# andreaskoepf/faster-rcnn.torch

Measured on AMD Instinct MI355X. Metric: images/sec (vgg_small 800x450 fwd+bwd), higher is better.
Workload: dtype f32 (conv / Linear(13824,1024) operands as 2 x fp16 split planes: 22 significand bits, 3 MFMA partial products; fp32 accumulate)

## Files before the change

### faster-rcnn.torch_amd/csrc/convx.hip

```cpp
#include <cstdlib>

#include "kernels.h"
#include "amax.h"
#include <type_traits>
#ifdef CX_TRACE
#include <cstdio>
#include <vector>
#endif

namespace frcnn {

typedef float f32x16 __attribute__((ext_vector_type(16)));
typedef __bf16 bf16x8 __attribute__((ext_vector_type(8)));
typedef __bf16 bf16x2 __attribute__((ext_vector_type(2)));
typedef float f32x2 __attribute__((ext_vector_type(2)));
typedef _Float16 f16x8 __attribute__((ext_vector_type(8)));
typedef _Float16 f16x2 __attribute__((ext_vector_type(2)));

#define CX_BM 128
#define CX_CH 16
#define CX_OCC 3
#define CX_PP 204
constexpr int cx_pp(int k) { return k == 3 ? CX_PP : k == 5 ? 240 : 308; }
#define CX_NA 2
// ... 946 lines not shown
  int grid = a.tilesX * a.tilesY * a.mTiles * a.splitK;
  if (grid > AMAX_MAX_BLOCKS) a.amax_out = nullptr;
#ifdef CX_TRACE
  static unsigned long long* tbuf = nullptr;
  const char* tfile = getenv("FRCNN_X3_TRACE");
  if (tfile && !tbuf) FR_HIP(hipMalloc(&tbuf, 8192 * 512));
  a.trace = tfile && grid <= 8192 ? tbuf : nullptr;
  if (a.trace) FR_HIP(hipMemsetAsync(tbuf, 0, (size_t)grid * 512, s));
#endif
  double bytes = 4.0 * ((double)a.Cin * a.H * a.W + (double)a.M * a.Ho * a.Wo);
  const size_t lds = std::max<size_t>((size_t)cx_ring(NP) * (2 * NP * 64 * WM * 16) + (size_t)CX_NB * (2 * NP * cx_pp(KS) * 16), a.wide ? 4 * 64 * 32 * 4 : 0);
  FR_LAUNCH(KC_CONV_X3, flops, bytes, s, (conv_x3_kernel<KS, WM, SLOPE, SCALE, EPI, NP>), dim3(grid), dim3(256), lds, a);
  FR_LAUNCH_CHECK();
#ifdef CX_TRACE
  if (a.trace) {
    FR_HIP(hipStreamSynchronize(s));
    std::vector<unsigned long long> hst((size_t)grid * 64);
    FR_HIP(hipMemcpy(hst.data(), tbuf, hst.size() * 8, hipMemcpyDeviceToHost));
    if (FILE* f = fopen(tfile, "w")) {
      fprintf(f, "# grid %d M %d Cin %d Ho %d Wo %d TH %d TW %d splitK %d wide %d WM %d EPI %d\n", grid, a.M, a.Cin, a.Ho, a.Wo, a.TH, a.TW, a.splitK, a.wide, WM, EPI);
      for (int b = 0; b < grid; ++b) {
        for (int j = 0; j < 64; ++j) fprintf(f, "%llu ", hst[(size_t)b * 64 + j]);
        fprintf(f, "\n");
      }
      fclose(f);
    }
  }
#endif
  return FRCNN_OK;
}

int conv_x3(const float* in, int Cin, int H, int W, const float* in_slope, const float* in_scale, const void* wp,
            const float* bias, int M, int k, int pad, float* out, int out_mode, double algo_flops, hipStream_t s, int ws_slot,
            const X3PostAct* post, const float* amax_in, const float* amax_w, float* amax_out) {
  FR_CHECK((k == 3 || k == 5 || k == 7) && Cin % CX_CH == 0 && M % 64 == 0,
           "conv_x3: %d channels -> %d filters, %dx%d is not a split-bf16 shape", Cin, M, k, k);
  FR_CHECK((double)Cin * H * W * 4.0 < 4294967295.0, "conv_x3: input tensor too large for 32-bit offsets");
  CxArgs a;
  a.in = in; a.in_slope = in_slope; a.in_scale = in_scale; a.wp = wp; a.bias = bias; a.out = out;
  a.amax_in = amax_in; a.amax_w = amax_w; a.amax_out = amax_out;
  const bool f16 = amax_in != nullptr;
  FR_CHECK(!f16 || amax_w, "conv_x3: the two-plane fp16 form needs the magnitudes of both tensors");
  a.Cin = Cin; a.H = H; a.W = W; a.M = M; a.pad = pad;
  a.Ho = H + 2 * pad - k + 1; a.Wo = W + 2 * pad - k + 1;
  FR_CHECK(a.Ho > 0 && a.Wo > 0, "conv_x3: empty output (%dx%d, k=%d, pad=%d)", H, W, k, pad);
  x3_choose_tile(a.Ho, a.Wo, k, &a.TH, &a.TW);
  a.tilesX = cdiv(a.Wo, a.TW); a.tilesY = cdiv(a.Ho, a.TH);
  const int bm = conv_x3_bm(M, a.Ho, a.Wo, k);
  a.mTiles = M / bm;
  a.nChunks = Cin / CX_CH;
  const long blocks = (long)a.tilesX * a.tilesY * a.mTiles;
  const int min_chunks = cdiv(36, k * k);
  const long slots = 256 * (k == 3 ? CX_OCC : 2);
  int splitK = (int)std::min<long>(std::min<long>(std::max<long>(1, slots / blocks), k == 3 ? 16 : 24), std::max(1, a.nChunks / min_chunks));
  a.chunksPerSplit = cdiv(a.nChunks, splitK);
  a.splitK = cdiv(a.nChunks, a.chunksPerSplit);
  a.out_mode = out_mode;
  a.post = post ? *post : X3PostAct{nullptr, nullptr, nullptr, nullptr};
  a.wide = 0;
  FR_CHECK(!post || (k == 3 && out_mode == OUT_STORE && !in_slope && !in_scale && !bias && post->x && post->slope),
           "conv_x3: the fused activation backward belongs to a storing 3x3 input-gradient launch");
  bool slab = false;
  if (a.splitK > 1) {
    float* ws = nullptr;
    FR_TRY(x3_workspace((size_t)a.splitK * M * a.Ho * a.Wo * 4, &ws, ws_slot & 7));
    a.out = ws; a.out_mode = 3; a.bias = nullptr; slab = true;
    a.amax_out = nullptr;
  }
  a.wide = a.Wo % 4 == 0 && a.TW % 4 == 0 && ((uintptr_t)a.out & 15) == 0 &&
           (!post || ((uintptr_t)post->x & 15) == 0);
  if (algo_flops <= 0) algo_flops = 2.0 * M * Cin * k * k * (double)a.Ho * a.Wo;
  int rc;
  const int act = (in_slope ? 2 : 0) | (in_scale ? 1 : 0);
  if (f16 && k != 3) {
    FR_CHECK(act == 0 && bm == 128, "conv_x3: a %dx%d launch takes no fused input activation and 128-filter blocks", k, k);
    rc = k == 5 ? launch_x3<5, 2, false, false, 0, 2>(a, algo_flops, s) : launch_x3<7, 2, false, false, 0, 2>(a, algo_flops, s);
  } else if (f16) {
    if (post && a.splitK == 1)
      rc = bm == 128 ? launch_x3<3, 2, false, false, 1, 2>(a, algo_flops, s) : launch_x3<3, 1, false, false, 1, 2>(a, algo_flops, s);
    else if (bm == 128)
      rc = act == 3 ? launch_x3<3, 2, true, true, 0, 2>(a, algo_flops, s) : act == 2 ? launch_x3<3, 2, true, false, 0, 2>(a, algo_flops, s)
         : act == 1 ? launch_x3<3, 2, false, true, 0, 2>(a, algo_flops, s) : launch_x3<3, 2, false, false, 0, 2>(a, algo_flops, s);
    else
      rc = act == 3 ? launch_x3<3, 1, true, true, 0, 2>(a, algo_flops, s) : act == 2 ? launch_x3<3, 1, true, false, 0, 2>(a, algo_flops, s)
         : act == 1 ? launch_x3<3, 1, false, true, 0, 2>(a, algo_flops, s) : launch_x3<3, 1, false, false, 0, 2>(a, algo_flops, s);
  } else if (post && a.splitK == 1) {
    rc = bm == 128 ? launch_x3<3, 2, false, false, 1>(a, algo_flops, s) : launch_x3<3, 1, false, false, 1>(a, algo_flops, s);
  } else if (k == 3 && bm == 128) {
    rc = act == 3 ? launch_x3<3, 2, true, true>(a, algo_flops, s) : act == 2 ? launch_x3<3, 2, true, false>(a, algo_flops, s)
       : act == 1 ? launch_x3<3, 2, false, true>(a, algo_flops, s) : launch_x3<3, 2, false, false>(a, algo_flops, s);
  } else if (k == 3) {
    rc = act == 3 ? launch_x3<3, 1, true, true>(a, algo_flops, s) : act == 2 ? launch_x3<3, 1, true, false>(a, algo_flops, s)
       : act == 1 ? launch_x3<3, 1, false, true>(a, algo_flops, s) : launch_x3<3, 1, false, false>(a, algo_flops, s);
  } else {
    FR_CHECK(act == 0 && bm == 128, "conv_x3: a %dx%d launch takes no fused input activation and 128-filter blocks", k, k);
    rc = k == 5 ? launch_x3<5, 2, false, false>(a, algo_flops, s) : launch_x3<7, 2, false, false>(a, algo_flops, s);
  }
  FR_TRY(rc);
  if (amax_out && !slab && (long)a.tilesX * a.tilesY * a.mTiles > AMAX_MAX_BLOCKS)
    FR_TRY(tensor_absmax(out, (long)M * a.Ho * a.Wo, amax_out, s));
  if (slab) {
    long total = (long)M * a.Ho * a.Wo;
    int grid;
    const long hw = (long)a.Ho * a.Wo;
    const X3PostAct pa = post ? *post : X3PostAct{nullptr, nullptr, nullptr, nullptr};
    const bool al = ((uintptr_t)out & 15) == 0 && ((uintptr_t)a.out & 15) == 0 && (!post || ((uintptr_t)post->x & 15) == 0);
    const int vec = al && hw % 4 == 0 ? 4 : al && hw % 2 == 0 ? 2 : 1;
    grid = (int)std::min<long>(cdivl(total / vec, 256), 4096);
    if (vec == 4)
      FR_LAUNCH(KC_ELEMWISE, 0, total * 4.0 * (a.splitK + 1), s, x3_splitk_reduce_kernel<4>, dim3(grid), dim3(256), 0,
                (const float*)a.out, a.splitK, M, hw, bias, out, out_mode == OUT_ADD ? 1 : 0, pa, amax_out);
    else if (vec == 2)
      FR_LAUNCH(KC_ELEMWISE, 0, total * 4.0 * (a.splitK + 1), s, x3_splitk_reduce_kernel<2>, dim3(grid), dim3(256), 0,
                (const float*)a.out, a.splitK, M, hw, bias, out, out_mode == OUT_ADD ? 1 : 0, pa, amax_out);
    else
      FR_LAUNCH(KC_ELEMWISE, 0, total * 4.0 * (a.splitK + 1), s, x3_splitk_reduce_kernel<1>, dim3(grid), dim3(256), 0,
                (const float*)a.out, a.splitK, M, hw, bias, out, out_mode == OUT_ADD ? 1 : 0, pa, amax_out);
    FR_LAUNCH_CHECK();
  }
  return FRCNN_OK;
}

}
```

### faster-rcnn.torch_amd/csrc/elem.hip

```cpp
#include <algorithm>

#include <mutex>
#include <unordered_map>

#include "kernels.h"
#include "amax.h"

namespace frcnn {

__device__ __forceinline__ float wave_sum(float v) {
#pragma unroll
  for (int o = 32; o > 0; o >>= 1) v += __shfl_down(v, o, 64);
  return v;
}

__device__ __forceinline__ float block_sum(float v, float* sh) {
  v = wave_sum(v);
  const int lane = threadIdx.x & 63, w = threadIdx.x >> 6;
  if (lane == 0) sh[w] = v;
  __syncthreads();
  float r = 0.f;
  if (threadIdx.x < 64) {
    r = threadIdx.x < (blockDim.x >> 6) ? sh[threadIdx.x] : 0.f;
    r = wave_sum(r);
// ... 285 lines not shown
  *out = e.first;
  return FRCNN_OK;
}

static int act_bwd_chunks(int C, long hw) {
  long want = cdivl(512, C);
  long maxc = cdivl(hw, 4096);
  return (int)std::max<long>(1, std::min<long>(want, maxc));
}

int maxpool_act_backward(const float* gpool, const unsigned char* idx, const float* x, int C, int H,
                         int W, const float* slope, const float* scale, float* gx, float* gbias,
                         float* gslope, hipStream_t s, float* amax) {
  int Ho = (H - 2 + 1) / 2 + 1, Wo = (W - 2 + 1) / 2 + 1;
  int chunks = act_bwd_chunks(C, (long)H * W);
  float* const amax_after = (amax && (long)C * chunks > AMAX_MAX_BLOCKS) ? amax : nullptr;
  if (amax_after) amax = nullptr;
  float *pb = nullptr, *pa = nullptr;
  if (deterministic()) { FR_TRY(det_workspace(s, (size_t)2 * C * chunks, &pb)); pa = pb + (size_t)C * chunks; }
  const bool vec = (W % 4 == 0) && (Wo % 2 == 0) && (((uintptr_t)gpool | (uintptr_t)x | (uintptr_t)gx) % 16 == 0) &&
                   ((uintptr_t)idx % 2 == 0);
  if (vec)
    FR_LAUNCH(KC_ELEMWISE, 0, (double)C * H * W * 9.25, s, (act_backward_kernel<true, true>), dim3(C * chunks),
              dim3(ACT_BWD_THREADS), 0, gpool, idx, x, C, H, W, Ho, Wo, slope, scale, gx, gbias, gslope, chunks, pb, pa, amax);
  else
    FR_LAUNCH(KC_ELEMWISE, 0, (double)C * H * W * 9.25, s, (act_backward_kernel<true, false>), dim3(C * chunks),
              dim3(ACT_BWD_THREADS), 0, gpool, idx, x, C, H, W, Ho, Wo, slope, scale, gx, gbias, gslope, chunks, pb, pa, amax);
  FR_LAUNCH_CHECK();
  if (pb) FR_TRY(fold_partials(gbias ? pb : nullptr, (slope && gslope) ? pa : nullptr, C, chunks, gbias, gslope, s));
  if (amax_after) FR_TRY(tensor_absmax(gx, (long)C * H * W, amax_after, s));
  return FRCNN_OK;
}

int act_backward(const float* gy, const float* x, int C, long hw, const float* slope,
                 const float* scale, float* gx, float* gbias, float* gslope, hipStream_t s, float* amax) {
  int chunks = act_bwd_chunks(C, hw);
  float* const amax_after = (amax && (long)C * chunks > AMAX_MAX_BLOCKS) ? amax : nullptr;
  if (amax_after) amax = nullptr;
  float *pb = nullptr, *pa = nullptr;
  if (deterministic()) { FR_TRY(det_workspace(s, (size_t)2 * C * chunks, &pb)); pa = pb + (size_t)C * chunks; }
  const bool vec = (hw % 4 == 0) && (((uintptr_t)gy | (uintptr_t)x | (uintptr_t)gx) % 16 == 0);
  if (vec)
    FR_LAUNCH(KC_ELEMWISE, 0, (double)C * hw * 12.0, s, (act_backward_kernel<false, true>), dim3(C * chunks),
              dim3(ACT_BWD_THREADS), 0, gy, (const unsigned char*)nullptr, x, C, 1, (int)hw, 1, 1, slope, scale, gx,
              gbias, gslope, chunks, pb, pa, amax);
  else
    FR_LAUNCH(KC_ELEMWISE, 0, (double)C * hw * 12.0, s, (act_backward_kernel<false, false>), dim3(C * chunks),
              dim3(ACT_BWD_THREADS), 0, gy, (const unsigned char*)nullptr, x, C, 1, (int)hw, 1, 1, slope, scale, gx,
              gbias, gslope, chunks, pb, pa, amax);
  FR_LAUNCH_CHECK();
  if (pb) FR_TRY(fold_partials(gbias ? pb : nullptr, (slope && gslope) ? pa : nullptr, C, chunks, gbias, gslope, s));
  if (amax_after) FR_TRY(tensor_absmax(gx, (long)C * hw, amax_after, s));
  return FRCNN_OK;
}

__global__ void channel_sum_kernel(const float* __restrict__ g, long hw, float* gbias, int chunks, float* part_b) {
  __shared__ float sh[16];
  const int c = blockIdx.x / chunks, chunk = blockIdx.x % chunks;
  long per = cdivl(hw, chunks);
  per = (per + 3) & ~3L;
  const long beg = chunk * per, end = beg + per < hw ? beg + per : hw;
  const float* gc = g + (size_t)c * hw;
  float sb = 0.f;
  if (beg < end) {
    if ((reinterpret_cast<uintptr_t>(gc + beg) & 15) == 0) {
      const long n4 = (end - beg) >> 2;
// ... 586 lines not shown
```

### faster-rcnn.torch_amd/csrc/kernels.h

```cpp
#pragma once
#include <algorithm>

#include "common.h"

namespace frcnn {

int conv_cc(int k);
int conv_mpad(int M);
size_t conv_pack_floats(int Kchan, int M, int k);
int conv_pack_weights(const float* w, int O, int C, int k, float* wf, float* wd, hipStream_t s);
struct PackJob { long w_off; long total; float* dst; int O, C, k, mode, Mpad, blk_begin, nblk; };
PackJob conv_pack_job(long w_off, int O, int C, int k, int mode, float* dst);
int conv_pack_assign_blocks(PackJob* jobs, int njobs, int total_blocks);
int conv_pack_weights_multi(const float* weights, const PackJob* jobs_dev, int njobs, int grid, hipStream_t s);

enum { OUT_STORE = 0, OUT_ADD = 1 };
struct IgemmPool { float* out; unsigned char* idx; const float* slope; const float* scale; float* amax = nullptr; };
int conv_igemm(const float* in, int Cin, int H, int W, const float* in_slope, const float* in_scale,
               const float* wp, const float* bias, int M, int k, int pad, float* out, int out_mode,
               double algo_flops, hipStream_t s, int ws_slot = 0,
               const IgemmPool* pool = nullptr, bool* pool_fused = nullptr);

void set_split_bf16(int on);
int get_split_bf16();
bool conv_x3_eligible(int Cin, int M, int k);
size_t conv_x3_pack_bytes(int Kchan, int M, int k);
struct PackXJob {
  long w_off; long total; void* dst; const float* amax; float* amax_w; int O, C, k, mode, bm, blk_begin, nblk;
  const int* oidx = nullptr; const int* cidx = nullptr; int Cs = 0; long bias_off = 0; float* bias_dst = nullptr;
};
PackXJob conv_x3_pack_job(long w_off, int O, int C, int k, int mode, void* dst, int Ho, int Wo);
int conv_x3_pack_assign_blocks(PackXJob* jobs, int njobs);
int conv_x3_pack_multi(const float* weights, const PackXJob* jobs_dev, int njobs, int grid, hipStream_t s);
int conv_x3_pack(const float* w, int O, int C, int k, int mode, void* dst, hipStream_t s, int Ho, int Wo,
                 const float* amax_rec_w = nullptr, float* amax_w = nullptr);
#define AMAX_REC 16400
#define AMAX_MAX_BLOCKS 16384
int tensor_absmax(const float* x, long n, float* rec, hipStream_t s);
struct AmaxJob { long off; long n; float* out; int blk_begin; };
int tensor_absmax_assign_blocks(AmaxJob* jobs, int njobs);
long tensor_absmax_record_floats(long n);
int tensor_absmax_multi(const float* w, const AmaxJob* jobs_dev, int njobs, int grid, hipStream_t s);
void set_x3_f16(int on);
int get_x3_f16();
int conv_x3(const float* in, int Cin, int H, int W, const float* in_slope, const float* in_scale, const void* wp,
            const float* bias, int M, int k, int pad, float* out, int out_mode, double algo_flops, hipStream_t s, int ws_slot = 0,
            const struct X3PostAct* post = nullptr, const float* amax_in = nullptr, const float* amax_w = nullptr,
            float* amax_out = nullptr);
struct X3PostAct {
  const float* x;
  const float* slope;
  const float* scale;
  float* gslope;
};

bool conv_wgradx_eligible(int Cin, int O, int k);
size_t conv_wgradx_workspace_bytes(int Cin, int H, int W, int O, int pad);
struct WgradMap { const int* omap = nullptr; const int* cmap = nullptr; int Cfull = 0; };
int conv_wgradx(const float* in, int Cin, int H, int W, const float* in_slope, const float* in_scale, const float* g, int O,
                int pad, float* gw, void* ws, size_t ws_bytes, hipStream_t s, float* gbias = nullptr,
                const float* amax_in = nullptr, const float* amax_g = nullptr,
                const WgradMap* map = nullptr);
int wgrad_reduce(const float* slab, int nSplit, int taps, int OC, float* gw, hipStream_t s);
int wgrad_reduce_map(const float* slab, int nSplit, int taps, int O, int C, float* gw, const WgradMap& map, hipStream_t s);
bool conv_wgrad_first_pooled_eligible(int Cin, int O, int k, int Wo);
int conv_wgrad_first_pooled(const float* in, int Cin, int H, int W, const float* gpool, const unsigned char* pidx, const float* x,
                            const float* slope, int O, int pad, float* gw, float* gbias, float* gslope, void* ws, size_t ws_bytes,
                            hipStream_t s);

size_t conv_wgrad_workspace_bytes(int Cin, int H, int W, int O, int k, int pad);
int conv_wgrad(const float* in, int Cin, int H, int W, const float* in_slope, const float* in_scale,
               const float* g, int O, int k, int pad, float* gw, void* ws, size_t ws_bytes, hipStream_t s,
               float* gbias = nullptr,
               const float* amax_in = nullptr, const float* amax_g = nullptr,
               const WgradMap* map = nullptr);

bool deterministic();
void set_deterministic(bool on);
int det_workspace(hipStream_t s, size_t floats, float** out);

int fill_zero(void* p, size_t bytes, hipStream_t s);
int scale_inplace(float* x, long n, float sc, hipStream_t s);
int add_inplace(float* y, const float* x, long n, hipStream_t s);
int act_forward(const float* x, int C, long hw, const float* slope, const float* scale, float* y,
                hipStream_t s);
int maxpool_act_forward(const float* x, int C, int H, int W, const float* slope, const float* scale,
                        float* out, unsigned char* idx, hipStream_t s, float* amax = nullptr);
// ... 191 lines not shown
```

### faster-rcnn.torch_amd/csrc/net.cpp

```cpp
#include <array>
#include <vector>
#include <cmath>
#include <cstring>

#include "kernels.h"

namespace frcnn {

static const int HEAD_OUT = 18;
static const int SPARSE_MAX_POS = 512;

struct DevBuf {
  void* p = nullptr;
  size_t bytes = 0;
  bool owned = true;
  void view(void* ptr, size_t n) { p = ptr; bytes = n; owned = false; }
  int ensure(size_t need) {
    if (need <= bytes) return FRCNN_OK;
    if (p && owned) (void)hipFree(p);
    owned = true;
    p = nullptr; bytes = 0;
    FR_HIP(hipMalloc(&p, need + 64));
    bytes = need;
    return FRCNN_OK;
// ... 48 lines not shown
  int in, n;
  bool bn;
  float p_drop;
  long w_off, b_off, bnw_off, bnb_off, a_off;
  DevBuf lin, pre, post, xhat, invstd, mask, g;
  DevBuf gin;
  DevBuf xp, xpT, gp, gpT;
  int x_form = 0;
  DevBuf am;
  const float* am_w_of = nullptr;
  long am_w_gen = -1;
};

}

using namespace frcnn;

static int g_drop_compact = -1;
static int drop_compact_on() {
  if (g_drop_compact < 0) g_drop_compact = getenv("FRCNN_DROP_COMPACT") ? (atoi(getenv("FRCNN_DROP_COMPACT")) != 0) : 1;
  return g_drop_compact;
}
static int pool_stream(int slot, hipStream_t* out) {
  static hipStream_t pool[8] = {};
  if (!pool[slot]) FR_HIP(hipStreamCreateWithFlags(&pool[slot], hipStreamNonBlocking));
  *out = pool[slot];
  return FRCNN_OK;
}

static int g_sparse_heads = -1;
static int sparse_heads_on() {
  if (g_sparse_heads < 0) g_sparse_heads = getenv("FRCNN_SPARSE_HEADS") ? (atoi(getenv("FRCNN_SPARSE_HEADS")) != 0) : 1;
  return g_sparse_heads;
}
static int g_static_weights = 0;
static long g_static_gen = 0;

struct frcnn_model {
  frcnn_model_desc d;
  std::vector<Conv> convs;
  std::vector<Block> blocks;
  std::vector<Head> heads;
  std::vector<ClsLayer> cls;
  long pnet_params = 0, total_params = 0;
  long bbox_w_off = 0, bbox_b_off = 0, clsw_off = 0, clsb_off = 0;
  int H = 0, W = 0;
  int training = 0;
  DevBuf delta_last;
  DevBuf zero_arena;
  size_t delta_bytes = 0, gpool_bytes = 0;
  DevBuf pack_jobs;
  DevBuf x3_jobs;
  DevBuf amax, amax_ws, amax_jobs;
  int n_amax = 0, n_amax_jobs = 0, amax_grid = 0;
  float* rec(int id) const { return (float*)amax.p + (size_t)id * AMAX_REC; }
  std::vector<unsigned char> am_live;
  float* rec_w(int id) { am_live[id] = 1; return rec(id); }
  void weights_live(bool heads_too) {
    for (auto& c : convs) if (c.x_f || c.x_d) am_live[c.am + 2] = 1;
    for (auto& hd : heads) if (heads_too && (hd.c3.x_f || hd.c3.x_d)) am_live[hd.c3.am + 2] = 1;
  }
  bool f16_packed = false;
  long eval_packs_gen = -1;
  const float* eval_packs_w = nullptr;
  int n_x3_all = 0, n_x3_fwd = 0, x3_grid_all = 0, x3_grid_fwd = 0;
  int n_pack_fwd = 0, n_pack_all = 0, n_pack_heads = 0, pack_grid_fwd = 0, pack_grid_all = 0, pack_grid_heads = 0;
// ... 528 lines not shown
  if (!m->upd_join_ev) FR_HIP(hipEventCreateWithFlags(&m->upd_join_ev, hipEventDisableTiming));
  return FRCNN_OK;
}
int frcnn_model_update_stream(frcnn_model* m, void** stream) {
  FR_CHECK(m && stream, "model_update_stream: null argument");
  FR_TRY(ensure_update_stream(m));
  m->update_armed = true;
  *stream = (void*)m->cw;
  return FRCNN_OK;
}
int frcnn_model_update_fork(frcnn_model* m, void* stream) {
  FR_CHECK(m != nullptr, "model_update_fork: null model");
  FR_TRY(ensure_update_stream(m));
  FR_HIP(hipEventRecord(m->upd_ev, S(stream)));
  FR_HIP(hipStreamWaitEvent(m->cw, m->upd_ev, 0));
  return FRCNN_OK;
}
int frcnn_model_update_join(frcnn_model* m, void* stream) {
  FR_CHECK(m != nullptr, "model_update_join: null model");
  FR_TRY(ensure_update_stream(m));
  FR_HIP(hipEventRecord(m->upd_join_ev, m->cw));
  FR_HIP(hipStreamWaitEvent(S(stream), m->upd_join_ev, 0));
  return FRCNN_OK;
}

int frcnn_get_option(const char* name, int* value) {
  FR_CHECK(name != nullptr && value != nullptr, "get_option: null argument");
  if (strcmp(name, "side_stream") == 0) { *value = side_enabled() ? 1 : 0; return FRCNN_OK; }
  if (strcmp(name, "gemm_x_roles") == 0) { *value = get_gemm_x_roles(); return FRCNN_OK; }
  if (strcmp(name, "deterministic") == 0) { *value = deterministic() ? 1 : 0; return FRCNN_OK; }
  if (strcmp(name, "static_weights") == 0) { *value = g_static_weights; return FRCNN_OK; }
  if (strcmp(name, "drop_compact") == 0) { *value = drop_compact_on(); return FRCNN_OK; }
  if (strcmp(name, "sparse_heads") == 0) { *value = sparse_heads_on(); return FRCNN_OK; }
  if (strcmp(name, "winograd") == 0) { *value = 0; return FRCNN_OK; }
  if (strcmp(name, "cnet_wgrad_async") == 0) { *value = g_cnet_wgrad_async; return FRCNN_OK; }
  if (strcmp(name, "split_bf16") == 0) { *value = get_split_bf16(); return FRCNN_OK; }
  if (strcmp(name, "x3_f16") == 0) { *value = get_x3_f16(); return FRCNN_OK; }
  FR_CHECK(false, "get_option: unknown option '%s'", name);
  return FRCNN_OK;
}

int frcnn_set_option(const char* name, int value) {
  FR_CHECK(name != nullptr, "set_option: null name");
  if (strcmp(name, "side_stream") == 0) { g_side_stream = value ? 1 : 0; return FRCNN_OK; }
  if (strcmp(name, "deterministic") == 0) { set_deterministic(value != 0); return FRCNN_OK; }
  if (strcmp(name, "static_weights") == 0) { g_static_weights = value != 0; ++g_static_gen; return FRCNN_OK; }
  if (strcmp(name, "drop_compact") == 0) { g_drop_compact = value != 0; return FRCNN_OK; }
  if (strcmp(name, "sparse_heads") == 0) { g_sparse_heads = value != 0; return FRCNN_OK; }
  if (strcmp(name, "gemm_x_roles") == 0) { set_gemm_x_roles(value); return FRCNN_OK; }
  if (strcmp(name, "split_bf16") == 0) { set_split_bf16(value); return FRCNN_OK; }
  if (strcmp(name, "x3_f16") == 0) { set_x3_f16(value); return FRCNN_OK; }
  if (strcmp(name, "winograd") == 0) return FRCNN_OK;
  if (strcmp(name, "cnet_wgrad_async") == 0) { g_cnet_wgrad_async = value ? 1 : 0; return FRCNN_OK; }
  FR_CHECK(false, "set_option: unknown option '%s'", name);
  return FRCNN_OK;
}

static int ensure_head_streams(frcnn_model* m);
static int ensure_side(frcnn_model* m) {
  if (!m->side) {
    FR_TRY(pool_stream(0, &m->side));
    FR_HIP(hipEventCreateWithFlags(&m->join_ev, hipEventDisableTiming));
    FR_HIP(hipEventCreateWithFlags(&m->loss_ev, hipEventDisableTiming));
    FR_HIP(hipEventCreateWithFlags(&m->chain_ev, hipEventDisableTiming));
    for (auto& h : m->heads) FR_HIP(hipEventCreateWithFlags(&h.done, hipEventDisableTiming));
  }
  return FRCNN_OK;
}

static int ensure_head_streams(frcnn_model* m) {
  static const int head_streams = getenv("FRCNN_HEAD_STREAMS") ? atoi(getenv("FRCNN_HEAD_STREAMS")) : 1;
  size_t hi = 0;
  for (auto& h : m->heads) {
    if (head_streams && hi < 5 && !h.stream) FR_TRY(pool_stream(2 + (int)hi, &h.stream));
    ++hi;
  }
  return FRCNN_OK;
}

static hipStream_t head_stream(frcnn_model* m, size_t i) { return m->heads[i].stream ? m->heads[i].stream : m->side; }
static int head_slot(frcnn_model* m, size_t i) { return m->heads[i].stream ? 2 + (int)(i % 5) : 1; }
// ... 330 lines not shown
    } break;
    case 4: {
      FR_CHECK(index >= 0 && index < (int)m->blocks.size() && m->H > 0 && m->blocks[index].has_drop, "debug_buffer: block %d has no dropout", index);
      const Block& k = m->blocks[index]; b = &k.scale; n = (size_t)m->d.filters[index] * 4;
    } break;
    case 1: {
      FR_CHECK(index >= 0 && index < (int)m->blocks.size() && m->H > 0, "debug_buffer: block %d (after a forward pass)", index);
      const Block& k = m->blocks[index]; b = &k.pidx; n = (size_t)m->d.filters[index] * k.Hp * k.Wp;
    } break;
    case 2: {
      FR_CHECK(index >= 0 && index < (int)m->heads.size() && m->H > 0, "debug_buffer: anchor net %d (after a forward pass)", index);
      const Conv& c = m->heads[index].c3; b = &c.x; n = (size_t)c.Cout * c.Ho * c.Wo * 4;
      if ((m->heads_sparse_fwd || m->heads_deferred) && m->last_w) {
        FR_HIP(hipDeviceSynchronize());
        if (!m->head_x3_fresh) { FR_TRY(refresh_group(m, m->last_w, (int)m->blocks.size(), nullptr)); m->head_x3_fresh = true; }
        FR_TRY(head_forward(m, m->heads[index], m->last_w, nullptr, 0));
        FR_HIP(hipDeviceSynchronize());
      }
    } break;
    case 3: {
      FR_CHECK(index >= 0 && index < (int)m->cls.size() && m->R > 0, "debug_buffer: classification layer %d (after frcnn_cnet_forward)", index);
      const ClsLayer& L = m->cls[index]; b = L.bn ? &L.pre : &L.lin; n = (size_t)m->R * L.n * 4;
    } break;
    case 7: case 11: {
      FR_CHECK(index >= 0 && index < (int)m->convs.size() && m->H > 0, "debug_buffer: backbone convolution %d (after a forward pass)", index);
      const Conv& c = m->convs[index];
      const Block& k = m->blocks[c.block];
      b = kind == 7 ? &c.x : &c.gx; n = (size_t)((k.dc_on && c.step == 0) ? k.nkM : c.Cout) * c.Ho * c.Wo * 4;
    } break;
    case 9: {
      FR_CHECK(index >= 0 && index < (int)m->blocks.size() && m->H > 0, "debug_buffer: block %d (after a forward pass)", index);
      const Block& k = m->blocks[index]; b = &k.pooled; n = (size_t)m->d.filters[index] * k.Hp * k.Wp * 4;
    } break;
    case 5: case 6: case 8: case 10: {
      const int nc = (int)m->convs.size();
      int id = -1;
      FR_CHECK(m->H > 0, "debug_buffer: magnitude records exist after a forward pass");
      if (kind == 6) {
        FR_CHECK(index >= 0 && index < (int)m->blocks.size(), "debug_buffer: block %d out of range", index);
        id = m->blocks[index].am;
      } else if (kind == 10) {
        FR_CHECK(index >= 0 && index < nc + (int)m->heads.size(), "debug_buffer: weight tensor %d out of range", index);
        id = (index < nc ? m->convs[index].am : m->heads[index - nc].c3.am) + 2;
      } else {
        FR_CHECK(index >= 0 && index < nc, "debug_buffer: backbone convolution %d out of range", index);
        id = m->convs[index].am + (kind == 8 ? 1 : 0);
      }
      FR_CHECK(id >= 0 && id < (int)m->am_live.size() && m->am_live[id], "debug_buffer: the last pass kept no magnitude record of kind %d, index %d", kind, index);
      *ptr = m->rec(id); *bytes = (long long)AMAX_REC * 4;
      return FRCNN_OK;
    }
    default: FR_CHECK(false, "debug_buffer: unknown kind %d", kind);
  }
  FR_CHECK(b->p && b->bytes >= n, "debug_buffer: buffer not allocated yet");
  *ptr = b->p; *bytes = (long long)n;
  return FRCNN_OK;
}

int frcnn_pnet_delta(frcnn_model* m, int i, float** ptr) {
  FR_CHECK(m->H > 0, "pnet_delta: call frcnn_pnet_forward first");
  FR_CHECK(i >= 1 && i <= (int)m->heads.size() + 1, "pnet_delta: index %d out of range", i);
  *ptr = i <= (int)m->heads.size() ? m->heads[i - 1].delta.f() : m->delta_last.f();
  return FRCNN_OK;
}

int frcnn_pnet_set_sparse_deltas(frcnn_model* m, int head, const int* positions, int count) {
// ... 416 lines not shown
      for (auto& h : m->heads) any = any || h.sp_count != 0;
      if (any) FR_TRY(heads_forward_dense(m, w, s));
      m->heads_deferred = false;
    }
    FR_TRY(join_side(m, s));
    if (backbone_trained(m)) FR_TRY(fill_zero((char*)m->zero_arena.p + m->delta_bytes, m->gpool_bytes, s));
    FR_TRY(backward_heads(m, w, grad, s, 0));
  }
  const int fb = m->frozen_blocks;
  if (fb < nb) {
    if (!m->train_heads) FR_TRY(fill_zero((char*)m->zero_arena.p + m->delta_bytes, m->gpool_bytes, s));
    Block& last = m->blocks.back();
    FR_TRY(add_inplace(last.gpooled.f(), m->delta_last.f(), (long)m->d.filters[nb - 1] * last.Hp * last.Wp, s));
  }
  if (m->update_armed) {
    if (!m->bwd_ev) FR_HIP(hipEventCreateWithFlags(&m->bwd_ev, hipEventDisableTiming));
    FR_HIP(hipEventRecord(m->bwd_ev, s));
  }
  for (int b = 0; b < fb; ++b) {
    while (m->block_ev.size() < (size_t)nb) {
      hipEvent_t e;
      FR_HIP(hipEventCreateWithFlags(&e, hipEventDisableTiming));
      m->block_ev.push_back(e);
    }
    FR_HIP(hipEventRecord(m->block_ev[b], s));
    FR_TRY(record_block_read(m, b, s));
  }
  const bool use_side = side_enabled();
  if (use_side) FR_TRY(ensure_side(m));
  hipStream_t ws = use_side ? m->side : s;
  size_t n_fork = 0;
  const bool fuse_act = !deterministic() && !(getenv("FRCNN_FUSE_ACT") && atoi(getenv("FRCNN_FUSE_ACT")) == 0);
  bool act_done = false;
  for (int b = nb - 1; b >= fb; --b) {
    Block& blk = m->blocks[b];
    for (int st = blk.nconv - 1; st >= 0; --st) {
      Conv& c = m->convs[blk.first_conv + st];
      const float* scale = (st == 0 && blk.has_drop) ? blk.scale.f() : nullptr;
      const bool fused_here = act_done;
      act_done = false;
      static const bool first_pooled_on = !(getenv("FRCNN_FIRST_POOLED") && atoi(getenv("FRCNN_FIRST_POOLED")) == 0);
      const bool first_pooled = fuse_act && first_pooled_on && b == 0 && st == 0 && blk.nconv == 1 && scale == nullptr &&
                                conv_wgrad_first_pooled_eligible(c.Cin, c.Cout, c.k, c.Wo);
      if (first_pooled) {
        FR_TRY(conv_wgrad_first_pooled(m->img.f(), c.Cin, c.H, c.W, blk.gpooled.f(), (const unsigned char*)blk.pidx.p, c.x.f(),
                                       w + c.a_off, c.Cout, c.pad, grad + c.w_off, grad + c.b_off, grad + c.a_off,
                                       m->wg_ws_first.p, m->wg_ws_first.bytes, s));
        while (m->block_ev.size() < (size_t)nb) {
          hipEvent_t e;
          FR_HIP(hipEventCreateWithFlags(&e, hipEventDisableTiming));
          m->block_ev.push_back(e);
        }
        FR_HIP(hipEventRecord(m->block_ev[b], s));
        FR_TRY(record_block_read(m, b, s));
        break;
      }
      if (fused_here) {
      } else if (st == blk.nconv - 1) {
        FR_TRY(maxpool_act_backward(blk.gpooled.f(), (const unsigned char*)blk.pidx.p, c.x.f(), c.Cout, c.Ho, c.Wo,
                                    w + c.a_off, scale, c.gx.f(), grad + c.b_off, grad + c.a_off, s,
                                    (c.x_d && m->f16_packed) ? m->rec_w(c.am + 1) : nullptr));
      } else {
        FR_TRY(act_backward(c.gx.f(), c.x.f(), c.Cout, (long)c.Ho * c.Wo, w + c.a_off, scale, c.gx.f(),
                            grad + c.b_off, grad + c.a_off, s, (c.x_d && m->f16_packed) ? m->rec_w(c.am + 1) : nullptr));
      }
      const float* in; const float* in_slope = nullptr; const float* in_scale = nullptr;
      if (st > 0) {
        Conv& pc = m->convs[blk.first_conv + st - 1];
        in = pc.x.f(); in_slope = w + pc.a_off;
        in_scale = (st - 1 == 0 && blk.has_drop) ? blk.scale.f() : nullptr;
      } else {
        in = b == 0 ? m->img.f() : m->blocks[b - 1].pooled.f();
      }
      const bool dc = blk.dc_on && st <= 1;
      int wg_cin = c.Cin, wg_o = c.Cout;
      WgradMap wmap;
      if (dc) {
        wmap.Cfull = c.Cin;
        if (st == 1) { wg_cin = blk.nkM; wmap.cmap = blk.dc_idx; in_scale = nullptr; }
        else { wg_o = blk.nkM; wmap.omap = blk.dc_idx; }
      }
      const float* wa_in = nullptr; const float* wa_g = nullptr;
      if (m->f16_packed && c.x_f && c.x_d && (st > 0 || b > 0)) {
        wa_in = st > 0 ? m->rec(m->convs[blk.first_conv + st - 1].am) : m->rec(m->blocks[b - 1].am);
        wa_g = m->rec(c.am + 1);
      }
      const bool on_caller = use_side && b == 0 && st == 0;
      if (use_side && !on_caller) FR_TRY(fork_side(m, s, n_fork++));
      if (on_caller) {
        FR_TRY(conv_wgrad(in, wg_cin, c.H, c.W, in_slope, in_scale, c.gx.f(), wg_o, c.k, c.pad, grad + c.w_off, m->wg_ws_first.p,
                          m->wg_ws_first.bytes, s, fused_here ? grad + c.b_off : nullptr, wa_in, wa_g, dc ? &wmap : nullptr));
        FR_HIP(hipEventRecord(m->join_ev, ws));
        FR_HIP(hipStreamWaitEvent(s, m->join_ev, 0));
      } else {
        FR_TRY(conv_wgrad(in, wg_cin, c.H, c.W, in_slope, in_scale, c.gx.f(), wg_o, c.k, c.pad, grad + c.w_off, m->wg_ws.p, m->wg_ws.bytes, ws,
                          fused_here ? grad + c.b_off : nullptr, wa_in, wa_g, dc ? &wmap : nullptr));
      }
      if (st == 0) {
        while (m->block_ev.size() < (size_t)nb) {
          hipEvent_t e;
          FR_HIP(hipEventCreateWithFlags(&e, hipEventDisableTiming));
          m->block_ev.push_back(e);
        }
        FR_HIP(hipEventRecord(m->block_ev[b], on_caller ? s : ws));
      }
      if (b == fb && st == 0) {
        FR_TRY(record_block_read(m, b, s));
        break;
      }
      float* gin = st > 0 ? m->convs[blk.first_conv + st - 1].gx.f() : m->blocks[b - 1].gpooled.f();
      const int gmode = st > 0 ? OUT_STORE : OUT_ADD;
      const float* ag = nullptr;
      const float* aw = nullptr;
      if (c.x_d && m->f16_packed) { ag = m->rec(c.am + 1); aw = m->amax_ws.f() + c.am; }
      const int dg_k = (dc && st == 0) ? blk.nkK : c.Cout, dg_m = (dc && st == 1) ? blk.nkM : c.Cin;
      const double fl = 2.0 * dg_k * dg_m * c.k * c.k * (double)c.Ho * c.Wo;
      if (c.x_d && st > 0 && fuse_act && c.k == 3) {
        Conv& pc = m->convs[blk.first_conv + st - 1];
        X3PostAct post{pc.x.f(), w + pc.a_off, (st - 1 == 0 && blk.has_drop && !dc) ? blk.scale.f() : nullptr, grad + pc.a_off};
        FR_TRY(conv_x3(c.gx.f(), dg_k, c.Ho, c.Wo, nullptr, nullptr, c.wxd.p, nullptr, dg_m, c.k, c.k - 1 - c.pad, gin, gmode, fl, s, 0, &post, ag, aw,
                       (pc.x_d && m->f16_packed) ? m->rec_w(pc.am + 1) : nullptr));
        act_done = true;
      } else if (c.x_d)
        FR_TRY(conv_x3(c.gx.f(), dg_k, c.Ho, c.Wo, nullptr, nullptr, c.wxd.p, nullptr, dg_m, c.k, c.k - 1 - c.pad, gin, gmode, fl, s, 0, nullptr, ag, aw));
      else
        FR_TRY(conv_igemm(c.gx.f(), c.Cout, c.Ho, c.Wo, nullptr, nullptr, c.wd.f(), nullptr, c.Cin, c.k,
                          c.k - 1 - c.pad, gin, gmode, fl, s));
      if (st == 0) FR_TRY(record_block_read(m, b, s));
    }
  }
  m->block_ev_valid = true;
  if (heads_tail && !m->heads_gin) FR_TRY(join_heads(m, s));
  FR_TRY(cw_join(m, s));
  if (use_side) {
    FR_HIP(hipEventRecord(m->join_ev, ws));
    FR_HIP(hipStreamWaitEvent(s, m->join_ev, 0));
    m->side_busy = false;
  }
  return FRCNN_OK;
}

static bool cnet_fuse() {
  const char* e = getenv("FRCNN_CNET_FUSE");
  return !(e && atoi(e) == 0);
}
static bool gemm_f16_on() {
  static const bool env_on = !(getenv("FRCNN_GEMM_F16") && atoi(getenv("FRCNN_GEMM_F16")) == 0);
  return env_on && get_x3_f16();
}
static int ensure_cnet(frcnn_model* m, int R) {
  for (auto& L : m->cls) {
    size_t n = (size_t)R * L.n * 4;
    FR_TRY(L.lin.ensure(n));
    if (L.bn) { FR_TRY(L.pre.ensure(n)); FR_TRY(L.xhat.ensure(n)); FR_TRY(L.invstd.ensure((size_t)L.n * 4)); }
    FR_TRY(L.post.ensure(n));
// ... 227 lines not shown
```

Before: 510.9.

## Fuse split-K slab reduction with maxpool and activation backward at block boundaries

```diff
diff --git a/faster-rcnn.torch_amd/csrc/convx.hip b/faster-rcnn.torch_amd/csrc/convx.hip
--- a/faster-rcnn.torch_amd/csrc/convx.hip
+++ b/faster-rcnn.torch_amd/csrc/convx.hip
@@ -1002,7 +1002,7 @@
 
 int conv_x3(const float* in, int Cin, int H, int W, const float* in_slope, const float* in_scale, const void* wp,
             const float* bias, int M, int k, int pad, float* out, int out_mode, double algo_flops, hipStream_t s, int ws_slot,
-            const X3PostAct* post, const float* amax_in, const float* amax_w, float* amax_out) {
+            const X3PostAct* post, const float* amax_in, const float* amax_w, float* amax_out, X3PoolBack* pool) {
   FR_CHECK((k == 3 || k == 5 || k == 7) && Cin % CX_CH == 0 && M % 64 == 0,
            "conv_x3: %d channels -> %d filters, %dx%d is not a split-bf16 shape", Cin, M, k, k);
   FR_CHECK((double)Cin * H * W * 4.0 < 4294967295.0, "conv_x3: input tensor too large for 32-bit offsets");
@@ -1030,6 +1030,8 @@
   a.wide = 0;
   FR_CHECK(!post || (k == 3 && out_mode == OUT_STORE && !in_slope && !in_scale && !bias && post->x && post->slope),
            "conv_x3: the fused activation backward belongs to a storing 3x3 input-gradient launch");
+  FR_CHECK(!pool || (!post && !bias && out_mode == OUT_ADD && a.Ho == (pool->H + 1) / 2 && a.Wo == (pool->W + 1) / 2),
+           "conv_x3: the pooling backward belongs behind an accumulating launch whose output is the pooled map's gradient");
   bool slab = false;
   if (a.splitK > 1) {
     float* ws = nullptr;
@@ -1074,6 +1076,11 @@
     int grid;
     const long hw = (long)a.Ho * a.Wo;
     const X3PostAct pa = post ? *post : X3PostAct{nullptr, nullptr, nullptr, nullptr};
+    if (pool && splitk_pool_backward_eligible(a.splitK, (const float*)a.out, out, *pool)) {
+      FR_TRY(splitk_pool_backward((const float*)a.out, a.splitK, M, out, *pool, s));
+      pool->done = true;
+      return FRCNN_OK;
+    }
     const bool al = ((uintptr_t)out & 15) == 0 && ((uintptr_t)a.out & 15) == 0 && (!post || ((uintptr_t)post->x & 15) == 0);
     const int vec = al && hw % 4 == 0 ? 4 : al && hw % 2 == 0 ? 2 : 1;
     grid = (int)std::min<long>(cdivl(total / vec, 256), 4096);
diff --git a/faster-rcnn.torch_amd/csrc/elem.hip b/faster-rcnn.torch_amd/csrc/elem.hip
--- a/faster-rcnn.torch_amd/csrc/elem.hip
+++ b/faster-rcnn.torch_amd/csrc/elem.hip
@@ -341,6 +341,119 @@
   return FRCNN_OK;
 }
 
+#ifndef POOL_FOLD_GROUP
+#define POOL_FOLD_GROUP 8
+#endif
+__global__ __launch_bounds__(ACT_BWD_THREADS) void splitk_pool_backward_kernel(const float* __restrict__ slab, int nSplit, long total,
+                                    float* __restrict__ gpool, const unsigned char* __restrict__ idx, const float* __restrict__ x,
+                                    int H, int W, int Hp, int Wp, const float* slope, const float* scale, float* __restrict__ gx,
+                                    float* gbias, float* gslope, int chunks, float* amax) {
+  __shared__ float sh[16];
+  __shared__ double shd[16];
+  float am = 0.f;
+  const int c = blockIdx.x / chunks, chunk = blockIdx.x % chunks;
+  const unsigned half = (unsigned)Wp >> 1, npair = (unsigned)Hp * half;
+  const unsigned per = (npair + chunks - 1) / chunks;
+  const unsigned beg = chunk * per, end = beg + per < npair ? beg + per : npair;
+  const float a = slope ? *slope : 1.f;
+  const float sc = scale ? scale[c] : 1.f;
+  const bool has_slope = slope != nullptr;
+  float sb = 0.f;
+  double sa = 0.0;
+  const size_t pofs = (size_t)c * Hp * Wp, fofs = (size_t)c * H * W;
+  const float* sl = slab + pofs;
+  float* gc = gpool + pofs;
+  const unsigned char* ic = idx + pofs;
+  const float* xc = x + fofs;
+  float* oc = gx + fofs;
+  const unsigned uW = (unsigned)W, uH = (unsigned)H, stride = blockDim.x;
+  auto place = [&](unsigned q, unsigned& i, bool& two) {
+    const unsigned oy = q / half, oxp = q - oy * half;
+    i = 2u * oy * uW + 4u * oxp;
+    two = 2u * oy + 1u < uH;
+  };
+  auto finish = [&](unsigned i, bool two, float2 v, unsigned ib, const float4& xa, const float4& xb) {
+    const float xr[2][4] = {{xa.x, xa.y, xa.z, xa.w}, {xb.x, xb.y, xb.z, xb.w}};
+#pragma unroll
+    for (int dy = 0; dy < 2; ++dy) {
+      if (dy == 1 && !two) break;
+      const unsigned code = (unsigned)dy * 2u;
+      float g[4];
+      g[0] = ((ib & 0xff) == code) ? v.x : 0.f;
+      g[1] = ((ib & 0xff) == code + 1) ? v.x : 0.f;
+      g[2] = ((ib >> 8) == code) ? v.y : 0.f;
+      g[3] = ((ib >> 8) == code + 1) ? v.y : 0.f;
+      float r[4];
+#pragma unroll
+      for (int j = 0; j < 4; ++j) {
+        float gj = g[j];
+        if (scale) gj *= sc;
+        r[j] = gj;
+        if (has_slope && !(xr[dy][j] > 0.f)) { r[j] = a * gj; sa += (double)xr[dy][j] * (double)gj; }
+        sb += r[j];
+        am = fmaxf(am, fabsf(r[j]));
+      }
+      *reinterpret_cast<float4*>(oc + i + (unsigned)dy * uW) = make_float4(r[0], r[1], r[2], r[3]);
+    }
+  };
+  for (unsigned q = beg + threadIdx.x; q < end; q += stride) {
+    unsigned i;
+    bool two;
+    place(q, i, two);
+    const float4 xa = *reinterpret_cast<const float4*>(xc + i);
+    const float4 xb = two ? *reinterpret_cast<const float4*>(xc + i + uW) : make_float4(1.f, 1.f, 1.f, 1.f);
+    const unsigned ib = *reinterpret_cast<const unsigned short*>(ic + 2u * q);
+    const float2 old = *reinterpret_cast<const float2*>(gc + 2u * q);
+    float2 v = make_float2(0.f, 0.f);
+    const float* sp = sl + 2u * q;
+    int s = 0;
+    for (; s + POOL_FOLD_GROUP <= nSplit; s += POOL_FOLD_GROUP) {
+      float2 p[POOL_FOLD_GROUP];
+#pragma unroll
+      for (int j = 0; j < POOL_FOLD_GROUP; ++j) p[j] = *reinterpret_cast<const float2*>(sp + (size_t)j * total);
+      sp += (size_t)POOL_FOLD_GROUP * total;
+#pragma unroll
+      for (int j = 0; j < POOL_FOLD_GROUP; ++j) { v.x += p[j].x; v.y += p[j].y; }
+    }
+    for (; s < nSplit; ++s, sp += total) {
+      const float2 p = *reinterpret_cast<const float2*>(sp);
+      v.x += p.x; v.y += p.y;
+    }
+    v.x += old.x; v.y += old.y;
+    *reinterpret_cast<float2*>(gc + 2u * q) = v;
+    finish(i, two, v, ib, xa, xb);
+  }
+  if (amax) amax_store_block(am, amax);
+  const float tb = block_sum(sb, sh);
+  if (threadIdx.x == 0 && gbias) unsafeAtomicAdd(gbias + c, tb);
+  if (slope && gslope) {
+    const float ta = (float)block_sum_d(sa, shd);
+    if (threadIdx.x == 0) unsafeAtomicAdd(gslope, ta);
+  }
+}
+
+bool splitk_pool_backward_eligible(int nSplit, const float* slab, const float* gpool, const X3PoolBack& p) {
+  const int Wp = (p.W - 2 + 1) / 2 + 1;
+  return nSplit > 1 && !deterministic() && p.W % 4 == 0 && Wp % 2 == 0 && (long)p.H * p.W < (1L << 31) &&
+         (((uintptr_t)slab | (uintptr_t)gpool | (uintptr_t)p.x | (uintptr_t)p.gx) % 16 == 0) && ((uintptr_t)p.idx % 2 == 0);
+}
+
+int splitk_pool_backward(const float* slab, int nSplit, int C, float* gpool, const X3PoolBack& p, hipStream_t s) {
+  FR_CHECK(splitk_pool_backward_eligible(nSplit, slab, gpool, p), "splitk_pool_backward: %d slabs of a %dx%d map's pooled gradient do not fit the fused fold",
+           nSplit, p.H, p.W);
+  const int Hp = (p.H - 2 + 1) / 2 + 1, Wp = (p.W - 2 + 1) / 2 + 1;
+  const int chunks = act_bwd_chunks(C, (long)p.H * p.W);
+  float* amax = p.amax;
+  float* const amax_after = (amax && (long)C * chunks > AMAX_MAX_BLOCKS) ? amax : nullptr;
+  if (amax_after) amax = nullptr;
+  const double bytes = (double)C * Hp * Wp * (4.0 * nSplit + 9.0) + (double)C * p.H * p.W * 8.0;
+  FR_LAUNCH(KC_ELEMWISE, 0, bytes, s, splitk_pool_backward_kernel, dim3(C * chunks), dim3(ACT_BWD_THREADS), 0, slab, nSplit,
+            (long)C * Hp * Wp, gpool, p.idx, p.x, p.H, p.W, Hp, Wp, p.slope, p.scale, p.gx, p.gbias, p.gslope, chunks, amax);
+  FR_LAUNCH_CHECK();
+  if (amax_after) FR_TRY(tensor_absmax(p.gx, (long)C * p.H * p.W, amax_after, s));
+  return FRCNN_OK;
+}
+
 int act_backward(const float* gy, const float* x, int C, long hw, const float* slope,
                  const float* scale, float* gx, float* gbias, float* gslope, hipStream_t s, float* amax) {
   int chunks = act_bwd_chunks(C, hw);
diff --git a/faster-rcnn.torch_amd/csrc/kernels.h b/faster-rcnn.torch_amd/csrc/kernels.h
--- a/faster-rcnn.torch_amd/csrc/kernels.h
+++ b/faster-rcnn.torch_amd/csrc/kernels.h
@@ -46,13 +46,29 @@
 int conv_x3(const float* in, int Cin, int H, int W, const float* in_slope, const float* in_scale, const void* wp,
             const float* bias, int M, int k, int pad, float* out, int out_mode, double algo_flops, hipStream_t s, int ws_slot = 0,
             const struct X3PostAct* post = nullptr, const float* amax_in = nullptr, const float* amax_w = nullptr,
-            float* amax_out = nullptr);
+            float* amax_out = nullptr,
+            struct X3PoolBack* pool = nullptr);
 struct X3PostAct {
   const float* x;
   const float* slope;
   const float* scale;
   float* gslope;
 };
+
+struct X3PoolBack {
+  const unsigned char* idx;
+  const float* x;
+  const float* slope;
+  const float* scale;
+  float* gx;
+  float* gbias;
+  float* gslope;
+  float* amax;
+  int H, W;
+  bool done = false;
+};
+bool splitk_pool_backward_eligible(int nSplit, const float* slab, const float* gpool, const X3PoolBack& p);
+int splitk_pool_backward(const float* slab, int nSplit, int C, float* gpool, const X3PoolBack& p, hipStream_t s);
 
 bool conv_wgradx_eligible(int Cin, int O, int k);
 size_t conv_wgradx_workspace_bytes(int Cin, int H, int W, int O, int pad);
diff --git a/faster-rcnn.torch_amd/csrc/net.cpp b/faster-rcnn.torch_amd/csrc/net.cpp
--- a/faster-rcnn.torch_amd/csrc/net.cpp
+++ b/faster-rcnn.torch_amd/csrc/net.cpp
@@ -104,6 +104,11 @@
 static int sparse_heads_on() {
   if (g_sparse_heads < 0) g_sparse_heads = getenv("FRCNN_SPARSE_HEADS") ? (atoi(getenv("FRCNN_SPARSE_HEADS")) != 0) : 1;
   return g_sparse_heads;
+}
+static int g_pool_x = -1;
+static int pool_x_on() {
+  if (g_pool_x < 0) g_pool_x = getenv("FRCNN_POOL_X") ? (atoi(getenv("FRCNN_POOL_X")) != 0) : 1;
+  return g_pool_x;
 }
 static int g_static_weights = 0;
 static long g_static_gen = 0;
@@ -698,6 +703,7 @@
   if (strcmp(name, "static_weights") == 0) { *value = g_static_weights; return FRCNN_OK; }
   if (strcmp(name, "drop_compact") == 0) { *value = drop_compact_on(); return FRCNN_OK; }
   if (strcmp(name, "sparse_heads") == 0) { *value = sparse_heads_on(); return FRCNN_OK; }
+  if (strcmp(name, "pool_x") == 0) { *value = pool_x_on(); return FRCNN_OK; }
   if (strcmp(name, "winograd") == 0) { *value = 0; return FRCNN_OK; }
   if (strcmp(name, "cnet_wgrad_async") == 0) { *value = g_cnet_wgrad_async; return FRCNN_OK; }
   if (strcmp(name, "split_bf16") == 0) { *value = get_split_bf16(); return FRCNN_OK; }
@@ -713,6 +719,7 @@
   if (strcmp(name, "static_weights") == 0) { g_static_weights = value != 0; ++g_static_gen; return FRCNN_OK; }
   if (strcmp(name, "drop_compact") == 0) { g_drop_compact = value != 0; return FRCNN_OK; }
   if (strcmp(name, "sparse_heads") == 0) { g_sparse_heads = value != 0; return FRCNN_OK; }
+  if (strcmp(name, "pool_x") == 0) { g_pool_x = value != 0; return FRCNN_OK; }
   if (strcmp(name, "gemm_x_roles") == 0) { set_gemm_x_roles(value); return FRCNN_OK; }
   if (strcmp(name, "split_bf16") == 0) { set_split_bf16(value); return FRCNN_OK; }
   if (strcmp(name, "x3_f16") == 0) { set_x3_f16(value); return FRCNN_OK; }
@@ -1109,6 +1116,10 @@
       FR_CHECK(index >= 0 && index < (int)m->blocks.size() && m->H > 0, "debug_buffer: block %d (after a forward pass)", index);
       const Block& k = m->blocks[index]; b = &k.pooled; n = (size_t)m->d.filters[index] * k.Hp * k.Wp * 4;
     } break;
+    case 12: {
+      FR_CHECK(index >= 0 && index < (int)m->blocks.size() && m->H > 0, "debug_buffer: block %d (after a forward pass)", index);
+      const Block& k = m->blocks[index]; b = &k.gpooled; n = (size_t)m->d.filters[index] * k.Hp * k.Wp * 4;
+    } break;
     case 5: case 6: case 8: case 10: {
       const int nc = (int)m->convs.size();
       int id = -1;
@@ -1591,6 +1602,15 @@
   size_t n_fork = 0;
   const bool fuse_act = !deterministic() && !(getenv("FRCNN_FUSE_ACT") && atoi(getenv("FRCNN_FUSE_ACT")) == 0);
   bool act_done = false;
+  const bool fold_pool = fuse_act && pool_x_on();
+  bool pool_done = false;
+  static const bool first_pooled_on = !(getenv("FRCNN_FIRST_POOLED") && atoi(getenv("FRCNN_FIRST_POOLED")) == 0);
+  auto first_pooled_case = [&](int b, int st) {
+    const Block& k = m->blocks[b];
+    const Conv& fc = m->convs[k.first_conv + st];
+    return fuse_act && first_pooled_on && b == 0 && st == 0 && k.nconv == 1 && !k.has_drop &&
+           conv_wgrad_first_pooled_eligible(fc.Cin, fc.Cout, fc.k, fc.Wo);
+  };
   for (int b = nb - 1; b >= fb; --b) {
     Block& blk = m->blocks[b];
     for (int st = blk.nconv - 1; st >= 0; --st) {
@@ -1598,9 +1618,9 @@
       const float* scale = (st == 0 && blk.has_drop) ? blk.scale.f() : nullptr;
       const bool fused_here = act_done;
       act_done = false;
-      static const bool first_pooled_on = !(getenv("FRCNN_FIRST_POOLED") && atoi(getenv("FRCNN_FIRST_POOLED")) == 0);
-      const bool first_pooled = fuse_act && first_pooled_on && b == 0 && st == 0 && blk.nconv == 1 && scale == nullptr &&
-                                conv_wgrad_first_pooled_eligible(c.Cin, c.Cout, c.k, c.Wo);
+      const bool pooled_here = pool_done;
+      pool_done = false;
+      const bool first_pooled = first_pooled_case(b, st);
       if (first_pooled) {
         FR_TRY(conv_wgrad_first_pooled(m->img.f(), c.Cin, c.H, c.W, blk.gpooled.f(), (const unsigned char*)blk.pidx.p, c.x.f(),
                                        w + c.a_off, c.Cout, c.pad, grad + c.w_off, grad + c.b_off, grad + c.a_off,
@@ -1615,6 +1635,7 @@
         break;
       }
       if (fused_here) {
+      } else if (pooled_here) {
       } else if (st == blk.nconv - 1) {
         FR_TRY(maxpool_act_backward(blk.gpooled.f(), (const unsigned char*)blk.pidx.p, c.x.f(), c.Cout, c.Ho, c.Wo,
                                     w + c.a_off, scale, c.gx.f(), grad + c.b_off, grad + c.a_off, s,
@@ -1680,6 +1701,15 @@
         FR_TRY(conv_x3(c.gx.f(), dg_k, c.Ho, c.Wo, nullptr, nullptr, c.wxd.p, nullptr, dg_m, c.k, c.k - 1 - c.pad, gin, gmode, fl, s, 0, &post, ag, aw,
                        (pc.x_d && m->f16_packed) ? m->rec_w(pc.am + 1) : nullptr));
         act_done = true;
+      } else if (c.x_d && st == 0 && fold_pool && c.k == 3 && !first_pooled_case(b - 1, m->blocks[b - 1].nconv - 1)) {
+        Block& pb = m->blocks[b - 1];
+        Conv& pc = m->convs[pb.first_conv + pb.nconv - 1];
+        X3PoolBack pool{(const unsigned char*)pb.pidx.p, pc.x.f(), w + pc.a_off, (pb.nconv == 1 && pb.has_drop) ? pb.scale.f() : nullptr,
+                        pc.gx.f(), grad + pc.b_off, grad + pc.a_off, (pc.x_d && m->f16_packed) ? m->rec_w(pc.am + 1) : nullptr,
+                        pc.Ho, pc.Wo};
+        FR_TRY(conv_x3(c.gx.f(), dg_k, c.Ho, c.Wo, nullptr, nullptr, c.wxd.p, nullptr, dg_m, c.k, c.k - 1 - c.pad, gin, gmode, fl, s, 0, nullptr, ag, aw,
+                       nullptr, &pool));
+        pool_done = pool.done;
       } else if (c.x_d)
         FR_TRY(conv_x3(c.gx.f(), dg_k, c.Ho, c.Wo, nullptr, nullptr, c.wxd.p, nullptr, dg_m, c.k, c.k - 1 - c.pad, gin, gmode, fl, s, 0, nullptr, ag, aw));
       else
```

After: 511.0, median of 2. About the same (+0.0%).
